# ml-jku/LRAM

Measured on AMD Instinct MI355X. Metric: env-steps/sec (action-inference), higher is better.
Workload: dtype f32

## Files before the change

lram_amd/csrc/engine.h:

```cpp
#pragma once
#include <algorithm>
#include <array>
#include <cstdlib>
#include <cstring>
#include <map>
#include <memory>
#include <string>
#include <vector>

#include "../../include/lram_hip.h"
#include "common.h"

namespace lram::host {

struct DevBuf {
  float* p = nullptr;
  size_t n = 0;
  void alloc(size_t numel) {
    release();
    if (numel == 0) return;
    LRAM_HIP_CHECK(hipMalloc(reinterpret_cast<void**>(&p), numel * sizeof(float)));
    n = numel;
  }
  void zero(hipStream_t s = nullptr) {
    if (p) LRAM_HIP_CHECK(hipMemsetAsync(p, 0, n * sizeof(float), s));
  }
  void release() {
    if (p) (void)hipFree(p);
    p = nullptr;
    n = 0;
  }
};

struct BlockWeights {
  const float *norm_g = nullptr, *norm_b = nullptr;
  const float *proj_up = nullptr, *conv_w = nullptr, *conv_b = nullptr, *wq = nullptr, *wk = nullptr, *wv = nullptr,
              *wi = nullptr, *bi = nullptr, *wf = nullptr, *bf = nullptr, *on_g = nullptr, *on_b = nullptr,
              *skip = nullptr, *proj_down = nullptr;
  const float *gate_w[4] = {nullptr, nullptr, nullptr, nullptr};
  const float *rt = nullptr, *rbias = nullptr, *gn_g = nullptr, *gn_b = nullptr, *ffn_norm_g = nullptr,
              *ffn_norm_b = nullptr, *ffn_up = nullptr, *ffn_down = nullptr;
  const float *in_proj = nullptr, *in_proj_b = nullptr, *x_proj = nullptr, *dt_proj = nullptr, *dt_bias = nullptr,
              *A_log = nullptr, *Dp = nullptr, *out_proj = nullptr, *out_proj_b = nullptr;
};

struct BlockState {
  DevBuf s0;
  DevBuf n;
  DevBuf m;
  DevBuf conv;
  DevBuf wk, wv;
  DevBuf coef;
  DevBuf gsc;
  DevBuf pw;
};

struct GraphKey {
  const void *obs, *rtg, *rew, *mask, *act, *tok;
  int emb, discrete, B;
  hipStream_t stream;
  bool operator==(const GraphKey& o) const {
    return obs == o.obs && rtg == o.rtg && rew == o.rew && mask == o.mask && act == o.act && tok == o.tok &&
           emb == o.emb && discrete == o.discrete && B == o.B && stream == o.stream;
  }
};

}

using namespace lram;
using namespace lram::host;

constexpr int kTokenTapMaxBatch = 1024;

struct lram_engine {
  lram_config cfg{};
  int device = 0;
  std::map<std::string, DevBuf> weights;
  bool finalized = false;
  std::vector<BlockWeights> bw;
  struct Split {
    uint16_t* p;
    size_t n;
  };
  std::map<const float*, Split> split;
  bool use_bf16x3 = true;
  bool use_f16x2 = true;
  int f16x2_min_rows = 256;
  struct Split16 {
    uint16_t* planes;
    float* inv;
    size_t rows, k;
  };
  std::map<const float*, Split16> split16;
  bool gemm_presplit = true;
  int64_t slstm_counts[3] = {0, 0, 0};
  double gemm_counts[8] = {0, 0, 0, 0, 0, 0, 0, 0};
  std::vector<DevBuf> slstm_rt2;
  std::vector<DevBuf> slstm_rinv;
  int lazy_cap2_envs = 896;
  std::map<const float*, DevBuf> narrow;
  bool gemm_narrow_on = true;
  int gemm_narrow_min_rows = 256;
  bool upz_beside = true;
  bool slstm_gates_one = true;
  bool gemm_narrow_f16 = true;
  bool gn_amax_handover = true;
  bool gn_planes = true;
  bool slstm_seq_f32 = false;
  bool slstm_seq = true;
  std::vector<DevBuf> gate_coef;
  bool front_multi = true;
  int front_min_envs = 256;
  std::vector<DevBuf> dt_wt;
  DevBuf ASCALE;
  size_t ascale_rows = 0;
  DevBuf AMX_XN, AMX_XA, AMX_H;
  const float *w_state = nullptr, *b_state = nullptr, *w_rtg = nullptr, *b_rtg = nullptr, *w_rew = nullptr,
              *b_rew = nullptr, *eln_g = nullptr, *eln_b = nullptr, *w_head = nullptr, *b_head = nullptr,
              *post_g = nullptr, *post_b = nullptr;
  struct ImgConv {
    const float *w = nullptr, *b = nullptr;
    int cin = 0, cout = 0;
  };
  ImgConv img_conv[3][5];
  const float *img_lin_w = nullptr, *img_lin_b = nullptr;
  int img_channels = 0, img_flat = 0;
  DevBuf IMG_P, IMG_X0, IMG_X1, IMG_T;
  DevBuf IMG_EMB;
  DevBuf IMG_FLAT, IMG_ROWS, IMG_LIST;
  int img_tile = 2048;
  int64_t img_counts[3] = {0, 0, 0};
  static constexpr int fold_bubbles_images = 8;
  bool slot_table = false;
  std::vector<uint8_t> slot_flags, slot_act;
  std::vector<int32_t> slot_img_prefix;
  uint8_t* slot_dev = nullptr;
  int32_t* slot_img_list = nullptr;
  int slot_n_image = 0;
  bool slot_has_discrete = false;
  int mask_words = 0;
  std::vector<uint32_t> mask_bits;
  uint32_t* mask_dev = nullptr;
  int mask_no_discrete_at = -1;
  static int mask_count_below(const uint32_t* bits, int words, int b, int n) {
    int cnt = 0;
    for (int k = 0; k < words && k * 32 < n; ++k) {
      const int left = n - k * 32;
      cnt += __builtin_popcount(bits[(size_t)b * words + k] & (left >= 32 ? 0xffffffffu : (1u << left) - 1u));
    }
    return cnt;
  }
  int mask_first_empty(const uint32_t* bits, int words, const uint8_t* flags) const {
    for (int b = 0; b < B; ++b) {
      const int n = (flags != nullptr && (flags[b] & 1)) ? cfg.n_discrete : cfg.n_vocab;
      if (mask_count_below(bits, words, b, n) == 0) return b;
    }
    return -1;
  }
  void drop_action_mask() {
    if (mask_dev) (void)hipFree(mask_dev);
    mask_dev = nullptr, mask_words = 0, mask_no_discrete_at = -1;
    mask_bits.clear();
  }
  int lazy_mode = 2;
  bool lazy = false;
  bool lazy_ready = false;
  int lazy_period = 13;
  int gn_fuse = 2;
  bool mamba_dt_fuse = true;
  int slstm_fused_rows = 512;
  int gemm_skinny_rows = 384;
  static constexpr int slstm_gates_rows = 768;
  int gemm_skinny_min = 5;
  static constexpr int gemm_skinny_k = 1024;
  static constexpr int fold_bubbles = 2;
  bool fold_tail = true;
  static constexpr int fold_tail_blocks = 2;
  struct Prefold {
    bool pending = false;
    int blocks = 0;
    int64_t step = 0;
    int period = 0, B = 0;
  } prefold;
  int64_t lazy_step = 0;
  std::vector<int> lazy_bound;
  bool lazy_dirty = false;
  DevBuf LZ_COUNT;
  std::vector<SlotSeg> slot_segs;
  SlotSeg* slot_segs_dev = nullptr;
  SlotChunk* slot_chunks_dev = nullptr;
  int slot_n_chunks = 0, slot_n_rec_chunks = 0;
  int32_t* slot_idx_dev = nullptr;
  std::vector<int64_t> slot_c_off;
  bool slot_y_checked = false;
  void drop_slot_segments() {
    if (slot_segs_dev) (void)hipFree(slot_segs_dev);
    if (slot_chunks_dev) (void)hipFree(slot_chunks_dev);
    if (slot_idx_dev) (void)hipFree(slot_idx_dev);
    slot_segs_dev = nullptr, slot_chunks_dev = nullptr, slot_idx_dev = nullptr;
    slot_segs.clear(), slot_c_off.clear();
    slot_n_chunks = slot_n_rec_chunks = 0;
  }
  int B = 0;
  int n_live = 0;
  int ctx_rows = 0;
  int context_rows() const { return ctx_rows == 0 ? B : n_live; }
  int64_t ctx_counts[4] = {0, 0, 0, 0};
  int64_t parked_dirty_step = 0;
  bool parked_windows_empty(int64_t step) const { return step - parked_dirty_step >= (int64_t)lazy_period; }
  std::vector<BlockState> st;
  DevBuf X, XN, TOK, HID, U, Q, K, V, XA, H, G, SCAL, RY, LOGITS, RES, DTP;
  DevBuf XN2;
  DevBuf GATES, AMAT, VEC;
  DevBuf SEQ_EMB;
  DevBuf CTX, KEEP;
  DevBuf SCORE_LG;
  int score_rows = 4096;
  static constexpr int kScoreMinRows = 16;
  int last_head = -1;
  int tok_cap = 0;
  bool chunk_prefill = true;
  bool chunk_exact_fp32 = false;
  bool chunk_lanes = true;
  static constexpr int kMaxLanes = 3;
  static constexpr int n_lanes = 3;
  DevBuf twin[kMaxLanes - 1][21];
  std::vector<hipEvent_t> lane_ev[kMaxLanes];
  DevBuf SK;
  static constexpr size_t kSplitKSlotElems = 6u << 20;
  static constexpr int kSplitKSlots = 9;
  size_t ucols = 0, icols = 0;
  bool graph_mode = false;
  bool graph_valid = false;
  GraphKey graph_key{};
  hipGraph_t graph = nullptr;
  hipGraphExec_t graph_exec = nullptr;
  hipStream_t capture_stream = nullptr;
  int n_micro = 0;
  int compat_repeat = 1;
  DevBuf X0, U0;
  bool compat_share = true;
  bool compat_stale = false;
  bool sampling = false;
  SampleArgs sample;
  uint64_t* sample_draw = nullptr;
  std::vector<SampleSlot> sample_slots;
  SampleSlot* sample_slots_dev = nullptr;
  int sslot_k_max = 0, sslot_k_at = -1, sslot_kd_max = 0, sslot_kd_at = -1;
  void sample_slot_maxima() {
    sslot_k_max = sslot_kd_max = 0, sslot_k_at = sslot_kd_at = -1;
    for (size_t b = 0; b < sample_slots.size(); ++b) {
      const SampleSlot& t = sample_slots[b];
      if (t.mode == 0) continue;
      if (t.top_k > sslot_k_max) sslot_k_max = t.top_k, sslot_k_at = (int)b;
      if (slot_table && b < slot_flags.size() && (slot_flags[b] & 1) && t.top_k > sslot_kd_max)
        sslot_kd_max = t.top_k, sslot_kd_at = (int)b;
    }
  }
  void drop_sample_slots() {
    if (sample_slots_dev) (void)hipFree(sample_slots_dev);
    sample_slots_dev = nullptr;
    sample_slots.clear();
    sample_slot_maxima();
  }
  static constexpr int cell_unroll = 16;
// ... 207 lines not shown
```

lram_amd/csrc/engine.hip:

```cpp
#include "engine.h"

namespace {

const float* need(lram_engine* e, const std::string& name, size_t numel) {
  auto it = e->weights.find(name);
  if (it == e->weights.end()) throw Error("lram: missing weight '" + name + "'");
  if (it->second.n != numel)
    throw Error("lram: weight '" + name + "' has " + std::to_string(it->second.n) + " elements, expected " +
                std::to_string(numel));
  return it->second.p;
}
const float* optional(lram_engine* e, const std::string& name, size_t numel) {
  auto it = e->weights.find(name);
  if (it == e->weights.end()) return nullptr;
  if (it->second.n != numel)
    throw Error("lram: weight '" + name + "' has " + std::to_string(it->second.n) + " elements, expected " +
                std::to_string(numel));
  return it->second.p;
}

void validate_config(const lram_config& c) {
  LRAM_REQUIRE(c.abi_version == LRAM_ABI_VERSION, "config.abi_version does not match the library");
  LRAM_REQUIRE(c.backbone == LRAM_BACKBONE_XLSTM || c.backbone == LRAM_BACKBONE_MAMBA, "unknown backbone");
  LRAM_REQUIRE(c.d_model > 0 && c.d_model % 4 == 0 && c.d_model <= 2048, "d_model must be a multiple of 4, <= 2048");
// ... 326 lines not shown
                        (size_t)e->B * c.n_heads * (kChunkMaxTokens + 3) * kChunkMaxTokens * 4;
    if (want > have + free_b - std::min<size_t>(free_b, (size_t)2 << 30)) return seq;
    alloc_workspace(e, kChunkMaxTokens);
    LRAM_HIP_CHECK(hipDeviceSynchronize());
  }
  return steps;
}

}

namespace {

bool lazy_geometry_ok(const lram_engine* e) {
  return has_mlstm_block(e) && mlstm_lazy_supported(e->cfg.inner / e->cfg.n_heads, e->cfg.tokens_per_step);
}

void slot_segments_build(lram_engine* e) {
  e->drop_slot_segments();
  if (e->B <= 0) return;
  const lram_config& c = e->cfg;
  const int64_t B = e->B;
  std::vector<SlotSeg>& segs = e->slot_segs;
  int64_t rec = 0;
  const int64_t rec_numel = lram_state_bytes_per_env(e) / 4;
  auto add = [&](float* base, int64_t stride, int64_t numel, int kind, int parity, bool in_record) {
    if (base == nullptr || numel <= 0) return;
    SlotSeg sg{};
    sg.base = base, sg.stride = stride, sg.numel = (int32_t)numel, sg.kind = kind, sg.parity = parity;
    sg.rec_off = in_record ? rec : -1;
    const bool slot_ok = numel % 4 == 0 && stride % 4 == 0 && (reinterpret_cast<uintptr_t>(base) & 15) == 0;
    const bool rec_ok = in_record && rec % 4 == 0 && rec_numel % 4 == 0;
    sg.vec = (slot_ok ? 1 : 0) | (slot_ok && rec_ok ? 2 : 0);
    if (in_record) rec += numel;
    segs.push_back(sg);
  };
  e->slot_c_off.assign(c.n_blocks, -1);
  e->slot_y_checked = false;
  for (int i = 0; i < c.n_blocks; ++i) {
    BlockState& s = e->st[i];
    if (c.backbone == LRAM_BACKBONE_MAMBA) {
      add(s.s0.p, (int64_t)c.d_inner * c.d_state, (int64_t)c.d_inner * c.d_state, kSlotSegState, -1, true);
      add(s.conv.p, (int64_t)c.d_inner * c.d_conv, (int64_t)c.d_inner * c.d_conv, kSlotSegState, -1, true);
    } else if (c.block_is_slstm[i]) {
      const int64_t D = c.d_model;
      const bool checked = e->slstm_rinv.size() > (size_t)i && e->slstm_rinv[i].p != nullptr;
      e->slot_y_checked = e->slot_y_checked || checked;
      for (int p = 0; p < 4; ++p)
        add(s.s0.p + p * B * D, D, D, p == 0 && checked ? kSlotSegSlstmY : kSlotSegState, -1, true);
      add(s.conv.p, (int64_t)c.conv_k * D, (int64_t)c.conv_k * D, kSlotSegState, -1, true);
    } else {
      const int64_t NH = c.n_heads, DH = e->dh();
      e->slot_c_off[i] = rec;
      add(s.s0.p, NH * DH * DH, NH * DH * DH, kSlotSegC, -1, true);
      add(s.n.p, c.inner, c.inner, kSlotSegState, -1, true);
      add(s.m.p, NH, NH, kSlotSegState, -1, true);
      add(s.conv.p, (int64_t)c.conv_k * c.inner, (int64_t)c.conv_k * c.inner, kSlotSegState, -1, true);
    }
  }
  LRAM_REQUIRE(rec == rec_numel, "slot state: the segment table does not add up to the record size");
  const size_t n_rec_segs = segs.size();
  if (e->lazy_ready) {
    const int64_t NH = c.n_heads, DH = e->dh(), W = kLazyWindow;
    for (int i = 0; i < c.n_blocks; ++i) {
      if (c.block_is_slstm[i]) continue;
      BlockState& s = e->st[i];
      add(s.wk.p, NH * W * DH, NH * W * DH, kSlotSegWindow, -1, false);
      add(s.wv.p, NH * W * DH, NH * W * DH, kSlotSegWindow, -1, false);
      for (int p = 0; p < 2; ++p) {
        add(s.coef.p + p * B * NH * W, NH * W, NH * W, kSlotSegCoef, p, false);
        add(s.gsc.p + p * B * NH, NH, NH, kSlotSegG, p, false);
      }
    }
    for (int p = 0; p < 2; ++p) add(e->LZ_COUNT.p + p * B, 1, 1, kSlotSegCount, p, false);
  }
  std::vector<SlotChunk> chunks;
  for (size_t k = 0; k < segs.size(); ++k) {
    if (k == n_rec_segs) e->slot_n_rec_chunks = (int)chunks.size();
    for (int32_t off = 0; off < segs[k].numel; off += kSlotChunk) chunks.push_back(SlotChunk{(int32_t)k, off});
  }
  if (segs.size() == n_rec_segs) e->slot_n_rec_chunks = (int)chunks.size();
  e->slot_n_chunks = (int)chunks.size();
  LRAM_HIP_CHECK(hipMalloc(reinterpret_cast<void**>(&e->slot_segs_dev), segs.size() * sizeof(SlotSeg)));
  LRAM_HIP_CHECK(hipMalloc(reinterpret_cast<void**>(&e->slot_chunks_dev), chunks.size() * sizeof(SlotChunk)));
  LRAM_HIP_CHECK(hipMalloc(reinterpret_cast<void**>(&e->slot_idx_dev), 2 * (size_t)B * sizeof(int32_t)));
  LRAM_HIP_CHECK(hipMemcpy(e->slot_segs_dev, segs.data(), segs.size() * sizeof(SlotSeg), hipMemcpyHostToDevice));
  LRAM_HIP_CHECK(hipMemcpy(e->slot_chunks_dev, chunks.data(), chunks.size() * sizeof(SlotChunk), hipMemcpyHostToDevice));
}

void lazy_alloc(lram_engine* e) {
  if (e->lazy_ready || e->B <= 0 || !lazy_geometry_ok(e)) return;
  const lram_config& c = e->cfg;
  const size_t B = e->B, NH = c.n_heads, DH = e->dh();
  for (int i = 0; i < c.n_blocks; ++i) {
    if (c.block_is_slstm[i]) continue;
    BlockState& s = e->st[i];
    s.wk.alloc(B * NH * kLazyWindow * DH);
    s.wv.alloc(B * NH * kLazyWindow * DH);
    s.coef.alloc(2 * B * NH * kLazyWindow);
    s.gsc.alloc(2 * B * NH);
    if (!mlstm_lazy_fused_scores((int)DH)) {
      s.pw.alloc(B * NH * 4 * kLazyWT);
      s.pw.zero();
    }
    s.coef.zero();
  }
  e->LZ_COUNT.alloc(2 * B);
  e->LZ_COUNT.zero();
  for (int i = 0; i < c.n_blocks; ++i) {
    if (c.block_is_slstm[i]) continue;
    BlockState& s = e->st[i];
    for (int p = 0; p < 2; ++p)
      launch_mlstm_lazy_clear(reinterpret_cast<int32_t*>(e->LZ_COUNT.p) + p * B, s.gsc.p + p * B * NH, nullptr, (int)B,
                              (int)NH, nullptr);
  }
  LRAM_HIP_CHECK(hipDeviceSynchronize());
  e->lazy_step = 0;
  e->parked_dirty_step = 0;
  e->prefold = lram_engine::Prefold{};
  e->lazy_ready = true;
  slot_segments_build(e);
}

bool lazy_choice(const lram_engine* e) {
  if (e->lazy_mode == 0 || !lazy_geometry_ok(e)) return false;
  if (e->lazy_mode == 1) return true;
  return mlstm_block_bytes(e) >= 128.0 * 1024 * 1024;
}

struct Knob {
  const char* name;
  void (*set)(lram_engine& e, const char* v);
};
const Knob kKnobs[] = {
    {"LRAM_STATE", [](lram_engine& e, const char* v) {
       const std::string m(v);
       e.lazy_mode = m == "lazy" ? 1 : (m == "eager" || m == "materialised" || m == "materialized") ? 0 : 2;
     }},
    {"LRAM_LAZY_PERIOD", [](lram_engine& e, const char* v) { e.lazy_period = std::max(1, std::min(14, std::atoi(v))); }},
    {"LRAM_LAZY_CAP2_ENVS", [](lram_engine& e, const char* v) { e.lazy_cap2_envs = std::max(0, std::atoi(v)); }},
    {"LRAM_FOLD_TAIL", [](lram_engine& e, const char* v) { e.fold_tail = std::atoi(v) != 0; }},
    {"LRAM_GN_FUSE", [](lram_engine& e, const char* v) { e.gn_fuse = std::max(0, std::min(2, std::atoi(v))); }},
    {"LRAM_F16_MIN_ROWS", [](lram_engine& e, const char* v) { e.f16x2_min_rows = std::max(9, std::atoi(v)); }},
    {"LRAM_GEMM_PRESPLIT", [](lram_engine& e, const char* v) { e.gemm_presplit = std::atoi(v) != 0; }},
    {"LRAM_GEMM_NARROW", [](lram_engine& e, const char* v) { e.gemm_narrow_on = std::atoi(v) != 0, e.gemm_narrow_f16 = std::atoi(v) != 2; }},
    {"LRAM_UPZ_8P", [](lram_engine& e, const char* v) { e.upz_beside = std::atoi(v) != 0; }},
    {"LRAM_SLSTM_GATES_ONE", [](lram_engine& e, const char* v) { e.slstm_gates_one = std::atoi(v) != 0; }},
    {"LRAM_GN_AMAX", [](lram_engine& e, const char* v) { e.gn_amax_handover = std::atoi(v) != 0, e.gn_planes = std::atoi(v) >= 2; }},
    {"LRAM_GEMM_SKINNY_ROWS", [](lram_engine& e, const char* v) { e.gemm_skinny_rows = std::max(0, std::atoi(v)); }},
    {"LRAM_GEMM_SKINNY_MIN", [](lram_engine& e, const char* v) { e.gemm_skinny_min = std::max(1, std::atoi(v)); }},
    {"LRAM_SLSTM_FUSED_ROWS", [](lram_engine& e, const char* v) { e.slstm_fused_rows = std::max(0, std::atoi(v)); }},
    {"LRAM_SLSTM_SEQ", [](lram_engine& e, const char* v) { e.slstm_seq = std::atoi(v) != 0, e.slstm_seq_f32 = std::atoi(v) == 2; }},
    {"LRAM_FRONT_MULTI", [](lram_engine& e, const char* v) { e.front_multi = std::atoi(v) != 0; }},
    {"LRAM_FRONT_MIN_ENVS", [](lram_engine& e, const char* v) { e.front_min_envs = std::max(1, std::atoi(v)); }},
    {"LRAM_MAMBA_DT_FUSE", [](lram_engine& e, const char* v) { e.mamba_dt_fuse = std::atoi(v) != 0; }},
    {"LRAM_COMPAT_SHARE", [](lram_engine& e, const char* v) { e.compat_share = std::atoi(v) != 0; }},
    {"LRAM_PREFILL_CHUNK", [](lram_engine& e, const char* v) {
       e.chunk_prefill = std::atoi(v) != 0, e.chunk_exact_fp32 = std::atoi(v) == 2, e.chunk_lanes = std::atoi(v) != 3;
     }},
    {"LRAM_SCORE_ROWS", [](lram_engine& e, const char* v) { e.score_rows = std::max(lram_engine::kScoreMinRows, std::atoi(v)); }},
    {"LRAM_IMG_TILE", [](lram_engine& e, const char* v) { e.img_tile = std::max(1, std::min(kConvMaxFrames, std::atoi(v))); }},
    {"LRAM_EVENT_SCOPE", [](lram_engine& e, const char* v) { e.event_device_scope = std::string(v) != "system"; }},
};

void state_alloc(lram_engine* e, int B) {
  LRAM_REQUIRE(e->finalized, "lram_finalize must be called before lram_state_alloc");
  LRAM_REQUIRE(B > 0 && B <= 65535, "batch must be in 1..65535");
  LRAM_HIP_CHECK(hipSetDevice(e->device));
  e->drop_graph();
  e->release_state();
  e->drop_slot_table();
  e->drop_sample_slots();
  e->drop_action_mask();
  const lram_config& c = e->cfg;
  const size_t D = c.d_model;
  e->st.resize(c.n_blocks);
  for (int i = 0; i < c.n_blocks; ++i) {
    BlockState& s = e->st[i];
    if (c.backbone == LRAM_BACKBONE_MAMBA) {
      s.s0.alloc((size_t)B * c.d_inner * c.d_state);
      s.conv.alloc((size_t)B * c.d_inner * c.d_conv);
    } else if (c.block_is_slstm[i]) {
      s.s0.alloc(4 * (size_t)B * D);
      s.conv.alloc((size_t)B * c.conv_k * D);
    } else {
      const size_t DH = e->dh();
      s.s0.alloc((size_t)B * c.n_heads * DH * DH);
      s.n.alloc((size_t)B * c.inner);
      s.m.alloc((size_t)B * c.n_heads);
      s.conv.alloc((size_t)B * c.conv_k * c.inner);
    }
    s.s0.zero();
    s.n.zero();
    s.m.zero();
    s.conv.zero();
  }
  e->B = B;
  e->n_live = B;
  e->ctx_rows = LRAM_CONTEXT_ROWS_ALL;
  alloc_workspace(e, kMaxTokens);
  e->lazy = lazy_choice(e);
  if (e->lazy) lazy_alloc(e);
  if (e->slot_segs_dev == nullptr) slot_segments_build(e);
  LRAM_HIP_CHECK(hipDeviceSynchronize());
}

}

extern "C" {

const char* lram_last_error(void) { return g_last_error.c_str(); }

int32_t lram_abi_version(void) { return LRAM_ABI_VERSION; }

int32_t lram_create(const lram_config* cfg, int32_t device, lram_engine** out) {
  return guarded([&] {
    LRAM_REQUIRE(cfg != nullptr && out != nullptr, "lram_create: null argument");
    validate_config(*cfg);
    int ndev = 0;
    LRAM_HIP_CHECK(hipGetDeviceCount(&ndev));
    LRAM_REQUIRE(device >= 0 && device < ndev, "lram_create: no such HIP device");
    LRAM_HIP_CHECK(hipSetDevice(device));
    auto e = std::make_unique<lram_engine>();
    e->cfg = *cfg;
    e->device = device;
    gemm_knobs_reload();
    for (const Knob& k : kKnobs)
      if (const char* v = std::getenv(k.name)) k.set(*e, v);
    *out = e.release();
  });
}

int32_t lram_destroy(lram_engine* e) {
  return guarded([&] {
    if (e) {
      (void)hipSetDevice(e->device);
      delete e;
    }
  });
}

int32_t lram_set_weight(lram_engine* e, const char* name, const float* host_data, size_t numel) {
  return guarded([&] {
    LRAM_REQUIRE(e && name && host_data && numel > 0, "lram_set_weight: bad argument");
    LRAM_HIP_CHECK(hipSetDevice(e->device));
    DevBuf& b = e->weights[name];
    b.alloc(numel);
    LRAM_HIP_CHECK(hipMemcpy(b.p, host_data, numel * sizeof(float), hipMemcpyHostToDevice));
    e->finalized = false;
    e->drop_graph();
  });
}

int32_t lram_finalize(lram_engine* e) {
  return guarded([&] {
    LRAM_REQUIRE(e != nullptr, "lram_finalize: null engine");
    finalize(e);
  });
}

int32_t lram_state_alloc(lram_engine* e, int32_t batch) {
  return guarded([&] {
    LRAM_REQUIRE(e != nullptr, "lram_state_alloc: null engine");
    state_alloc(e, batch);
  });
}

int64_t lram_state_bytes_per_env(const lram_engine* e) {
  if (!e) return 0;
  const lram_config& c = e->cfg;
  int64_t elems = 0;
  for (int i = 0; i < c.n_blocks; ++i) {
    if (c.backbone == LRAM_BACKBONE_MAMBA) {
      elems += (int64_t)c.d_inner * (c.d_state + c.d_conv);
    } else if (c.block_is_slstm[i]) {
      elems += (int64_t)c.d_model * (4 + c.conv_k);
    } else {
      const int64_t DH = c.inner / c.n_heads;
      elems += (int64_t)c.n_heads * DH * DH + c.inner + c.n_heads + (int64_t)c.conv_k * c.inner;
    }
  }
  return elems * 4;
}

int32_t lram_set_graph_mode(lram_engine* e, int32_t enable) {
  return guarded([&] {
    LRAM_REQUIRE(e != nullptr, "lram_set_graph_mode: null engine");
    if (e->prefold.pending || (enable != 0 && e->lazy_ready)) {
      LRAM_HIP_CHECK(hipSetDevice(e->device));
      LRAM_HIP_CHECK(hipDeviceSynchronize());
      if (enable != 0)
        lazy_materialize(e, nullptr);
      else
        lazy_finish_prefold(e, nullptr);
      LRAM_HIP_CHECK(hipDeviceSynchronize());
    }
    e->graph_mode = enable != 0;
    if (!e->graph_mode) e->drop_graph();
  });
}

int32_t lram_set_state_mode(lram_engine* e, int32_t mode, int32_t fold_period) {
  return guarded([&] {
    LRAM_REQUIRE(e != nullptr, "lram_set_state_mode: null engine");
    LRAM_REQUIRE(mode >= 0 && mode <= 2, "lram_set_state_mode: mode must be 0 (materialised), 1 (lazy) or 2 (auto)");
    LRAM_REQUIRE(fold_period == 0 || (fold_period >= 1 && fold_period * e->cfg.tokens_per_step + 4 <= kLazyWindow),
                 "lram_set_state_mode: fold_period out of range (the window holds 48 tokens)");
// ... 158 lines not shown
```

lram_amd/csrc/engine_xlstm.hip:

```cpp
#include "engine.h"

namespace {

MlstmLazyArgs lazy_args(lram_engine* e, int i, int T, const uint8_t* reset, int b0, int nb, int step_off = 0) {
  const lram_config& c = e->cfg;
  const size_t NH = c.n_heads, DH = e->dh(), B = e->B;
  const int64_t step = e->lazy_step + step_off;
  const int in = (int)(step & 1), out = 1 - in;
  BlockState& st = e->st[i];
  MlstmLazyArgs a{};
  a.C = st.s0.p + (size_t)b0 * NH * DH * DH;
  a.wk = st.wk.p + (size_t)b0 * NH * kLazyWindow * DH;
  a.wv = st.wv.p + (size_t)b0 * NH * kLazyWindow * DH;
  a.coef_in = st.coef.p + (in * B + b0) * NH * kLazyWindow;
  a.coef_out = st.coef.p + (out * B + b0) * NH * kLazyWindow;
  a.g_in = st.gsc.p + (in * B + b0) * NH;
  a.g_out = st.gsc.p + (out * B + b0) * NH;
  a.count_in = reinterpret_cast<const int32_t*>(e->LZ_COUNT.p) + in * B + b0;
  a.count_out = reinterpret_cast<int32_t*>(e->LZ_COUNT.p) + out * B + b0;
  a.pw = st.pw.p ? st.pw.p + (size_t)b0 * NH * T * kLazyWT : nullptr;
  a.reset = reset ? reset + b0 : nullptr;
  a.B = nb, a.T = T, a.NH = (int)NH, a.DH = (int)DH;
  a.phase = (int)((step + b0) % e->lazy_period), a.period = e->lazy_period, a.force = 0;
  return a;
}

bool lazy_bound_compact(const lram_engine* e, int64_t step, int T) {
  const int P = e->lazy_period;
  if ((int)e->lazy_bound.size() != P) return false;
  const int c_due = lazy_due_class(step, P);
  for (int cls = 0; cls < P; ++cls)
    if (cls != c_due && e->lazy_bound[cls] + T > kLazyWindow) return false;
  return true;
}

void fold_block(lram_engine* e, int i, int T, const uint8_t* reset, bool compact, int step_off, hipStream_t s) {
  MlstmLazyArgs la = lazy_args(e, i, T, reset, 0, e->n_live, step_off);
  la.compact = compact ? 1 : 0;
  prof_record(e, s, true, true);
  launch_mlstm_lazy_fold(la, s);
  if (e->n_live < e->B && !e->parked_windows_empty(e->lazy_step + step_off)) {
    MlstmLazyArgs lp = lazy_args(e, i, T, nullptr, e->n_live, e->B - e->n_live, step_off);
    lp.compact = compact ? 2 : 0;
    launch_mlstm_lazy_fold(lp, s);
  }
  prof_record(e, s, false, true);
}

}

namespace lram::host {

void lazy_materialize(lram_engine* e, hipStream_t s) {
  lazy_finish_prefold(e, s);
  if (!e->lazy_ready || !e->lazy_dirty) return;
  const lram_config& c = e->cfg;
  const size_t B = e->B, NH = c.n_heads;
  for (int i = 0; i < c.n_blocks; ++i) {
    if (c.block_is_slstm[i]) continue;
    MlstmLazyArgs a = lazy_args(e, i, 1, nullptr, 0, e->B);
    a.force = 1;
    launch_mlstm_lazy_fold(a, s);
  }
  for (int i = 0; i < c.n_blocks; ++i) {
    if (c.block_is_slstm[i]) continue;
    for (int p = 0; p < 2; ++p)
      launch_mlstm_lazy_clear(reinterpret_cast<int32_t*>(e->LZ_COUNT.p) + p * B, e->st[i].gsc.p + p * B * NH, nullptr,
                              (int)B, (int)NH, s);
  }
  e->lazy_bound.assign(e->lazy_period, 0);
  e->lazy_dirty = false;
}

void lazy_finish_prefold(lram_engine* e, hipStream_t s) {
  if (!e->prefold.pending) return;
  const lram_engine::Prefold pf = e->prefold;
  e->prefold = lram_engine::Prefold{};
  LRAM_REQUIRE(e->lazy_ready && pf.B == e->B && pf.period == e->lazy_period && pf.step == e->lazy_step,
               "lazy mLSTM: a tail fold is pending for another state than the engine holds");
  const lram_config& c = e->cfg;
  const int B = e->B, NH = c.n_heads, P = e->lazy_period;
  const int side = (int)(e->lazy_step & 1);
  const int first = lazy_due_class(e->lazy_step, P);
  int k = 0;
  for (int i = 0; i < c.n_blocks; ++i) {
    if (c.block_is_slstm[i] || k++ < pf.blocks) continue;
    MlstmLazyArgs a = lazy_args(e, i, 1, nullptr, 0, B);
    a.compact = 1;
    launch_mlstm_lazy_fold(a, s);
  }
  int32_t* count = reinterpret_cast<int32_t*>(e->LZ_COUNT.p) + (size_t)side * B;
  for (int i = 0; i < c.n_blocks; ++i)
    if (!c.block_is_slstm[i]) launch_mlstm_lazy_folded(count, e->st[i].gsc.p + (size_t)side * B * NH, B, NH, first, P, s);
  launch_mlstm_lazy_folded(count, nullptr, B, NH, first, P, s);
  if ((int)e->lazy_bound.size() == P) e->lazy_bound[first] = 0;
}

}

namespace {

bool lean_front(const lram_engine* e, int T) {
  return lazy_active(e, T) && mlstm_lazy_fused_scores(e->cfg.inner / e->cfg.n_heads);
}

bool split_up_now(const lram_engine* e) { return e->n_live >= 2048 && !e->graph_mode; }

bool gn_fused(const lram_engine* e, int T) {
  const int dh = e->cfg.inner / e->cfg.n_heads;
  return (e->gn_fuse == 1 || (e->gn_fuse == 2 && e->n_live >= 2048)) && lean_front(e, T) && e->use_bf16x3 && (dh == 256 || dh == 128) && T <= 4 &&
         e->cfg.inner % 8 == 0 && e->cfg.d_model % 8 == 0 && e->n_live >= 64;
}

void mlstm_front(lram_engine* e, const Pass& pass, int i, int T, const uint8_t* reset, const Slice& sl) {
  const lram_config& c = e->cfg;
  const int D = c.d_model, inner = c.inner, NH = c.n_heads, rows = sl.nb * T;
  const size_t r0 = (size_t)sl.b0 * T, b0 = sl.b0;
  const BlockWeights& w = e->bw[i];
  BlockState& st = e->st[i];
  float* amx = e->use_f16x2 ? e->AMX_XN.p + r0 : nullptr;
  GemmArgs up;
  up.a = e->XN.p + r0 * D, up.lda = D, up.w = w.proj_up, up.ldw = D, up.c = e->U.p + r0 * e->ucols, up.ldc = 2 * inner;
  up.m = rows, up.n = split_up_now(e) ? inner : 2 * inner, up.k = D;
  if (gn_fused(e, T) && !split_up_now(e)) up.act_silu_from = inner;
  if (!split_up_now(e) && takes_skinny_with_norm(e, up)) {
    up.a = e->X.p + r0 * D, up.norm_g = w.norm_g, up.norm_b = w.norm_b, up.norm_eps = c.ln_eps, up.norm_rms = c.norm_is_rms;
    launch_gemm_skinny(up, sl.s);
    count_gemm(e, 3, up);
  } else {
    const bool ps = presplit_for(e, w.proj_up, rows, inner, D);
    uint16_t* xn2 = reinterpret_cast<uint16_t*>(e->XN2.p) + r0 * 32;
    const int64_t xn2_kt = ps ? (int64_t)(e->XN2.n / D) * 32 : 0;
    launch_row_norm(e->X.p + r0 * D, D, ps ? nullptr : e->XN.p + r0 * D, D, w.norm_g, w.norm_b, rows, D, c.ln_eps,
                    c.norm_is_rms, sl.s, nullptr, ps ? nullptr : amx, nullptr, ps ? xn2 : nullptr, (int64_t)e->XN2.n,
                    ps ? amx : nullptr, xn2_kt);
    up.a_amax = amx;
    if (ps) up.a = nullptr, up.a_amax = nullptr, up.a2 = xn2, up.a2_plane = (int64_t)e->XN2.n, up.a2_kt = xn2_kt, up.a2_inv = amx;
    if (pass.lane_rec != nullptr) up.beside_memory_bound = 2;
    gemm(e, up, sl.s);
  }
  if (e->front_multi && lean_front(e, T) && sl.nb >= e->front_min_envs && e->gate_coef[i].p != nullptr &&
      mlstm_front_supported(inner, NH, c.conv_k, T)) {
    MlstmFrontArgs fa;
    fa.u = e->U.p + r0 * e->ucols, fa.ldu = 2 * inner, fa.conv_state = st.conv.p + b0 * c.conv_k * inner;
    fa.n_state = st.n.p + b0 * inner, fa.m_state = st.m.p + b0 * NH;
    fa.conv_w = w.conv_w, fa.conv_b = w.conv_b, fa.wq = w.wq, fa.wk = w.wk, fa.gc = e->gate_coef[i].p, fa.bi = w.bi, fa.bf = w.bf;
    fa.xa = e->XA.p + r0 * e->icols, fa.scal = e->SCAL.p + r0 * NH * 4, fa.reset = reset ? reset + b0 : nullptr;
    fa.B = sl.nb, fa.T = T, fa.inner = inner, fa.NH = NH, fa.K = c.conv_k;
    LRAM_REQUIRE(pass.hold == nullptr, "mLSTM front end: the multi-env kernel has no hold rule (stored contexts run materialised)");
    launch_mlstm_front(fa, sl.s);
    return;
  }
  MlstmPreArgs pa;
  pa.u = e->U.p + r0 * e->ucols, pa.conv_state = st.conv.p + b0 * c.conv_k * inner, pa.n_state = st.n.p + b0 * inner;
  pa.m_state = st.m.p + b0 * NH;
  pa.conv_w = w.conv_w, pa.conv_b = w.conv_b, pa.wq = w.wq, pa.wk = w.wk, pa.wv = w.wv;
  pa.wi = w.wi, pa.bi = w.bi, pa.wf = w.wf, pa.bf = w.bf;
  pa.q = e->Q.p + r0 * e->icols, pa.k = e->K.p + r0 * e->icols, pa.v = e->V.p + r0 * e->icols;
  pa.xa = e->XA.p + r0 * e->icols;
  pa.scal = e->SCAL.p + r0 * NH * 4, pa.reset = reset ? reset + b0 : nullptr;
  pa.hold = pass.hold ? pass.hold + b0 : nullptr;
  pa.B = sl.nb, pa.T = T, pa.inner = inner, pa.NH = NH, pa.K = c.conv_k;
  pa.lean = lean_front(e, T) ? 1 : 0;
  if (T > kMaxTokens) {
    LRAM_REQUIRE(T <= e->tok_cap && e->AMAT.p != nullptr, "chunkwise prefill workspace not allocated");
    pa.gates = e->GATES.p + r0 * NH * 2;
    pa.amat = e->AMAT.p + b0 * NH * kChunkMaxTokens * kChunkMaxTokens;
    pa.vec = e->VEC.p + b0 * NH * 3 * kChunkMaxTokens;
  }
  launch_mlstm_pre(pa, sl.s);
}

void mlstm_up_z(lram_engine* e, int i, int T, const Slice& sl) {
  if (!split_up_now(e)) return;
  const lram_config& c = e->cfg;
  const int D = c.d_model, inner = c.inner, rows = sl.nb * T;
  const size_t r0 = (size_t)sl.b0 * T;
  GemmArgs up;
  up.a = e->XN.p + r0 * D, up.lda = D, up.w = e->bw[i].proj_up + (size_t)inner * D, up.ldw = D;
  up.c = e->U.p + r0 * e->ucols + inner, up.ldc = 2 * inner, up.m = rows, up.n = inner, up.k = D;
  if (e->use_f16x2) up.a_amax = e->AMX_XN.p + r0;
  if (presplit_for(e, e->bw[i].proj_up, rows, inner, D)) {
    up.a = nullptr, up.a_amax = nullptr;
    up.a2 = reinterpret_cast<uint16_t*>(e->XN2.p) + r0 * 32, up.a2_plane = (int64_t)e->XN2.n, up.a2_kt = (int64_t)(e->XN2.n / D) * 32;
    up.a2_inv = e->AMX_XN.p + r0;
  }
  if (gn_fused(e, T)) up.act_silu_from = 0;
  up.beside_memory_bound = e->upz_beside ? 1 : 0;
  gemm(e, up, sl.s);
}

void mlstm_cell(lram_engine* e, const Pass& pass, int i, int T, const uint8_t* reset, const Slice& sl, hipStream_t s) {
  const lram_config& c = e->cfg;
  const int inner = c.inner, NH = c.n_heads, DH = e->dh();
  const size_t r0 = (size_t)sl.b0 * T, b0 = sl.b0;
  MlstmCellArgs ca;
  ca.C = e->st[i].s0.p + b0 * NH * DH * DH, ca.q = e->Q.p + r0 * e->icols, ca.k = e->K.p + r0 * e->icols;
  ca.v = e->V.p + r0 * e->icols, ca.scal = e->SCAL.p + r0 * NH * 4, ca.h = e->H.p + r0 * e->icols;
  ca.reset = reset ? reset + b0 : nullptr, ca.B = sl.nb, ca.T = T, ca.NH = NH, ca.DH = DH;
  ca.hold = pass.hold ? pass.hold + b0 : nullptr;
  const long wgs = (long)sl.nb * NH * ((DH % 256 == 0) ? DH / 256 : (DH % 128 == 0) ? DH / 128 : DH / 64);
  ca.min_lds_bytes = wgs >= 1024 ? 84 * 1024 : 0;
  ca.unroll = e->cell_unroll;
  if (T > kMaxTokens) {
    ca.amat = e->AMAT.p + b0 * NH * kChunkMaxTokens * kChunkMaxTokens;
    ca.vec = e->VEC.p + b0 * NH * 3 * kChunkMaxTokens;
    ca.chunk_exact_fp32 = e->chunk_exact_fp32 ? 1 : 0;
  }
  prof_record(e, s, true);
  launch_mlstm_cell(ca, s);
  prof_record(e, s, false);
}

void mlstm_back(lram_engine* e, const Pass& pass, int i, int T, const Slice& sl) {
  const lram_config& c = e->cfg;
  const int D = c.d_model, inner = c.inner, NH = c.n_heads, DH = e->dh(), rows = sl.nb * T;
  const size_t r0 = (size_t)sl.b0 * T;
  const BlockWeights& w = e->bw[i];
  float* X = e->X.p + r0 * D;
  if (gn_fused(e, T)) {
    GemmArgs dn;
    dn.a = e->H.p + r0 * e->icols, dn.lda = inner, dn.w = w.proj_down, dn.ldw = inner, dn.c = X, dn.ldc = D, dn.residual = X;
    dn.m = rows, dn.n = D, dn.k = inner;
    dn.gate = e->U.p + r0 * e->ucols + inner, dn.ldg = 2 * inner;
    gemm(e, dn, sl.s);
    return;
  }
  GroupNormArgs ga;
  ga.h = e->H.p + r0 * e->icols, ga.gamma = w.on_g, ga.beta = w.on_b, ga.skip = w.skip, ga.xa = e->XA.p + r0 * e->icols;
  ga.u = e->U.p + r0 * e->ucols, ga.out = e->G.p + r0 * e->icols, ga.rows = rows, ga.NH = NH, ga.DH = DH, ga.mode = 0;
  ga.eps = c.ln_eps;
  const bool hand_over = e->gn_amax_handover && e->AMX_H.p != nullptr && f16x2_rows(e, rows, D, inner);
  GemmArgs dn;
  dn.a = e->G.p + r0 * e->icols, dn.lda = inner, dn.w = w.proj_down, dn.ldw = inner, dn.c = X, dn.ldc = D, dn.residual = X;
  dn.m = rows, dn.n = D, dn.k = inner;
  const int64_t bt = (int64_t)(e->G.n / e->icols);
  GemmArgs probe;
  const bool planes = hand_over && e->gn_planes && pass.n_slices == 1 && e->gemm_presplit && NH <= 8 && (inner & 31) == 0 && bt * inner * 4 < (1ll << 31) &&
                      f16x2_weight(e, w.proj_down, inner, &probe) && 4 * probe.w2_plane < (1ll << 31);
  if (planes) {
    ga.out = nullptr;
    ga.h2 = reinterpret_cast<uint16_t*>(e->G.p) + r0 * 32, ga.h2_plane = bt * inner, ga.h2_kt = bt * 32, ga.h2_inv = e->AMX_H.p + r0;
    dn.a = nullptr, dn.a2 = ga.h2, dn.a2_plane = ga.h2_plane, dn.a2_kt = ga.h2_kt, dn.a2_inv = ga.h2_inv;
  } else {
    ga.amax = hand_over ? e->AMX_H.p + r0 * NH : nullptr;
    if (hand_over) dn.a_amax = ga.amax, dn.amax_parts = NH;
  }
  launch_group_norm(ga, sl.s);
  gemm(e, dn, sl.s);
}

bool slstm_gates_one_bf16x3(const lram_engine* e, GemmArgs& g4, const BlockWeights& w, const float* XC, const float* XN, float* gates,
                            int Hs) {
  if (!e->use_bf16x3 || !e->slstm_gates_one) return false;
  int64_t plane = -1;
  for (int g = 0; g < 4; ++g) {
    auto it = e->split.find(w.gate_w[g]);
    if (it == e->split.end() || (plane >= 0 && (int64_t)it->second.n != plane)) return false;
    plane = (int64_t)it->second.n;
    g4.a_tab[g] = (g < 2) ? XC : XN, g4.w_tab[g] = w.gate_w[g], g4.c_tab[g] = gates + (int64_t)g * Hs;
    g4.w3_tab[g] = it->second.p;
  }
  g4.w3 = g4.w3_tab[0], g4.w3_plane = plane;
  return gemm_bf16x3_supported(g4) && !gemm_small_m(g4);
}

void slstm_block(lram_engine* e, const Pass& pass, int i, int T, const uint8_t* reset, const Slice& sl) {
  const lram_config& c = e->cfg;
  const int D = c.d_model, NH = c.n_heads, SDH = e->sdh(), F = c.ffn_dim, Hs = D, rows = sl.nb * T;
  const size_t r0 = (size_t)sl.b0 * T, b0 = sl.b0;
  const BlockWeights& w = e->bw[i];
  BlockState& st = e->st[i];
  hipStream_t s = sl.s;
  float* X = e->X.p + r0 * D;
  float* XN = e->XN.p + r0 * D;
  float* XC = e->Q.p + r0 * e->icols;
  float* gates = e->U.p + r0 * e->ucols;
  float* RY = e->RY.p + b0 * 4 * Hs;
  float* Y = e->H.p + r0 * e->icols;
  float* Ubuf = e->U.p + r0 * e->ucols;
  float* Gbuf = e->G.p + r0 * e->icols;
  float* state = st.s0.p + b0 * Hs;
  const uint8_t* hold = pass.hold ? pass.hold + b0 : nullptr;
  launch_row_norm(X, D, XN, D, w.norm_g, w.norm_b, rows, D, c.ln_eps, c.norm_is_rms, s);
  SlstmConvArgs sa;
  sa.xn = XN, sa.conv_state = st.conv.p + b0 * c.conv_k * D, sa.slstm_state = state, sa.conv_w = w.conv_w;
  sa.conv_b = w.conv_b, sa.xc = XC, sa.reset = reset ? reset + b0 : nullptr, sa.B = sl.nb, sa.T = T, sa.D = D;
  sa.K = c.conv_k, sa.state_B = e->B, sa.hold = hold;
  launch_slstm_conv(sa, s);
  GemmArgs g4;
  g4.a = XC, g4.lda = D, g4.sA1 = SDH, g4.w = w.gate_w[0], g4.ldw = SDH, g4.sW1 = (int64_t)SDH * SDH;
  g4.c = gates, g4.ldc = 4 * Hs, g4.sC1 = SDH, g4.m = rows, g4.n = SDH, g4.k = SDH, g4.nb1 = NH, g4.nb2 = 4;
  const bool gates_big = rows <= e->slstm_gates_rows && gemm_skinny_supported(g4) && g4.k <= 128;
  bool tab_aligned = true;
  for (int g = 0; g < 4; ++g)
    tab_aligned = tab_aligned && ((reinterpret_cast<uintptr_t>((g < 2) ? XC : XN) | reinterpret_cast<uintptr_t>(w.gate_w[g])) & 15) == 0;
  if (tab_aligned && (takes_skinny(e, g4) || gates_big)) {
    for (int g = 0; g < 4; ++g)
      g4.a_tab[g] = (g < 2) ? XC : XN, g4.w_tab[g] = w.gate_w[g], g4.c_tab[g] = gates + (int64_t)g * Hs;
    launch_gemm_skinny(g4, s);
    count_gemm(e, 3, g4);
// ... 225 lines not shown
```

lram_amd/csrc/mlstm_front.hip:

```cpp
#include <algorithm>
#include <cstdlib>

#include "common.h"
#include "device_math.h"
#include "xlstm_rules.h"

namespace lram {

namespace {

__global__ __launch_bounds__(256) void gate_coef_kernel(const float* wq, const float* wk, const float* wv, const float* wi,
                                                        const float* wf, int inner, int NH, float* gc) {
  const int gid = blockIdx.x * blockDim.x + threadIdx.x;
  const int ngroups = inner >> 2;
  if (gid >= ngroups * 2 * NH * 4) return;
  const int c = gid & 3, j = (gid >> 2) % (2 * NH), cg = gid / (8 * NH);
  const float* wg = (j < NH ? wi + (int64_t)j * 3 * inner : wf + (int64_t)(j - NH) * 3 * inner) + 4 * cg;
  double a = 0.0, b = 0.0;
  for (int o = 0; o < 4; ++o) {
    a += (double)wg[o] * (double)wq[(int64_t)cg * 16 + o * 4 + c] + (double)wg[inner + o] * (double)wk[(int64_t)cg * 16 + o * 4 + c];
    b += (double)wg[2 * inner + o] * (double)wv[(int64_t)cg * 16 + o * 4 + c];
  }
  gc[((int64_t)cg * 4 * NH + j) * 4 + c] = (float)a;
  gc[((int64_t)cg * 4 * NH + 2 * NH + j) * 4 + c] = (float)b;
}

template <int N, int M>
__device__ __forceinline__ void halve(const float* v, float* r, int lane) {
  const bool up = (lane & M) != 0;
#pragma unroll
  for (int i = 0; i < N; ++i) {
    const float send = up ? v[i] : v[i + N];
    const float keep = up ? v[i + N] : v[i];
    r[i] = keep + __shfl_xor(send, M, 64);
  }
}

constexpr int kNH = 4;
constexpr int kNG = 2 * kNH;

template <int T>
__global__ __launch_bounds__(256) void mlstm_front_kernel(MlstmFrontArgs a) {
  static_assert(T == 3, "the reduction tree below is laid out for 3 tokens x 8 gates");
  __shared__ float red[2][4][T * kNG];
  const int tid = threadIdx.x, lane = tid & 63, wave = tid >> 6;
  const int inner = 4 * 256, c0 = tid << 2, h = wave;
  const int e_begin = blockIdx.x * a.epw, e_end = min(a.B, e_begin + a.epw);
  if (e_begin >= e_end) return;

  float4 cw[4], wq[4], wk[4], gc[2 * kNG];
#pragma unroll
  for (int c = 0; c < 4; ++c) cw[c] = *reinterpret_cast<const float4*>(a.conv_w + (int64_t)(c0 + c) * 4);
  const float4 cb = *reinterpret_cast<const float4*>(a.conv_b + c0);
#pragma unroll
  for (int o = 0; o < 4; ++o) {
    wq[o] = *reinterpret_cast<const float4*>(a.wq + (int64_t)tid * 16 + o * 4);
    wk[o] = *reinterpret_cast<const float4*>(a.wk + (int64_t)tid * 16 + o * 4);
  }
#pragma unroll
  for (int j = 0; j < 2 * kNG; ++j) gc[j] = *reinterpret_cast<const float4*>(a.gc + ((int64_t)tid * 2 * kNG + j) * 4);
  const float bias_i = a.bi[h], bias_f = a.bf[h];
  const float sqrt_dh = 16.f;

  float4 win[4], nst, xm[T];
  float m_in;
  unsigned rsb;
  const uint8_t* rbase = a.reset != nullptr ? a.reset : reinterpret_cast<const uint8_t*>(a.conv_w);
  auto request = [&](int b) {
#pragma unroll
    for (int k = 0; k < 4; ++k) win[k] = *reinterpret_cast<const float4*>(a.conv_state + ((int64_t)b * 4 + k) * inner + c0);
    nst = *reinterpret_cast<const float4*>(a.n_state + (int64_t)b * inner + c0);
#pragma unroll
    for (int t = 0; t < T; ++t) xm[t] = *reinterpret_cast<const float4*>(a.u + ((int64_t)b * T + t) * a.ldu + c0);
    m_in = a.m_state[(int64_t)b * kNH + h];
    rsb = rbase[a.reset != nullptr ? b : 0];
  };
  request(e_begin);

  for (int b = e_begin; b < e_end; ++b) {
    const int buf = (b - e_begin) & 1;
    const unsigned keep = (a.reset != nullptr && rsb != 0) ? 0u : 0xFFFFFFFFu;
    float4 w0 = masked4(win[0], keep), w1 = masked4(win[1], keep), w2 = masked4(win[2], keep), w3 = masked4(win[3], keep);
    float4 n = masked4(nst, keep);
    float m = masked(m_in, keep);
    const float4 x0 = xm[0], x1 = xm[1], x2 = xm[2];

    float4 q[T], k[T];
    float pg[T * kNG];
    auto token = [&](int t, const float4& p0, const float4& p1, const float4& p2, const float4& p3) {
      const float4 xa = conv4_silu(p0, p1, p2, p3, cw, cb);
      *reinterpret_cast<float4*>(a.xa + ((int64_t)b * T + t) * inner + c0) = xa;
      q[t] = block4x4(wq, xa);
      k[t] = block4x4(wk, xa);
#pragma unroll
      for (int j = 0; j < kNG; ++j) pg[t * kNG + j] = dot4(gc[j], xa) + dot4(gc[kNG + j], p3);
    };
    token(0, w1, w2, w3, x0);
    token(1, w2, w3, x0, x1);
    token(2, w3, x0, x1, x2);
    *reinterpret_cast<float4*>(a.conv_state + ((int64_t)b * 4 + 0) * inner + c0) = w3;
    *reinterpret_cast<float4*>(a.conv_state + ((int64_t)b * 4 + 1) * inner + c0) = x0;
    *reinterpret_cast<float4*>(a.conv_state + ((int64_t)b * 4 + 2) * inner + c0) = x1;
    *reinterpret_cast<float4*>(a.conv_state + ((int64_t)b * 4 + 3) * inner + c0) = x2;

    request(min(b + 1, e_end - 1));

    float r12[12], r6[6], r3[3];
    halve<12, 32>(pg, r12, lane);
    halve<6, 16>(r12, r6, lane);
    halve<3, 8>(r6, r3, lane);
#pragma unroll
    for (int i = 0; i < 3; ++i) {
      r3[i] += __shfl_xor(r3[i], 4, 64);
      r3[i] += __shfl_xor(r3[i], 2, 64);
      r3[i] += __shfl_xor(r3[i], 1, 64);
    }
    if ((lane & 7) == 0) {
      const int idx = ((lane & 32) ? 12 : 0) + ((lane & 16) ? 6 : 0) + ((lane & 8) ? 3 : 0);
#pragma unroll
      for (int i = 0; i < 3; ++i) red[buf][wave][idx + i] = r3[i];
    }
    __syncthreads();

    float f[T], ig[T], mt[T];
#pragma unroll
    for (int t = 0; t < T; ++t) {
      const float gi = red[buf][0][t * kNG + h] + red[buf][1][t * kNG + h] + red[buf][2][t * kNG + h] + red[buf][3][t * kNG + h] + bias_i;
      const float gf = red[buf][0][t * kNG + kNH + h] + red[buf][1][t * kNG + kNH + h] + red[buf][2][t * kNG + kNH + h] +
                       red[buf][3][t * kNG + kNH + h] + bias_f;
      const MlstmGate g = mlstm_gate_step(gi, gf, m);
      f[t] = g.f;
      ig[t] = g.i;
      mt[t] = m = g.m;
    }
    float d[T];
#pragma unroll
    for (int t = 0; t < T; ++t) {
      n = mlstm_n_step(n, f[t], ig[t], k[t], sqrt_dh);
      d[t] = wave_sum(dot4(q[t], n));
    }
    *reinterpret_cast<float4*>(a.n_state + (int64_t)b * inner + c0) = n;
    if (lane == 0) {
      a.m_state[(int64_t)b * kNH + h] = m;
#pragma unroll
      for (int t = 0; t < T; ++t) {
        *reinterpret_cast<float4*>(a.scal + (((int64_t)b * T + t) * kNH + h) * 4) =
            make_float4(f[t], ig[t], mlstm_denominator(d[t], mt[t]), mt[t]);
      }
    }
  }
}

}

bool mlstm_front_supported(int inner, int NH, int K, int T) { return inner == 1024 && NH == kNH && K == 4 && T == 3; }

void launch_gate_coef(const float* wq, const float* wk, const float* wv, const float* wi, const float* wf, int inner, int NH,
                      float* gc, hipStream_t stream) {
  const int n = (inner >> 2) * 2 * NH * 4;
  hipLaunchKernelGGL(gate_coef_kernel, dim3((unsigned)((n + 255) / 256)), dim3(256), 0, stream, wq, wk, wv, wi, wf, inner, NH, gc);
  LRAM_HIP_CHECK(hipGetLastError());
}

void launch_mlstm_front(const MlstmFrontArgs& a_in, hipStream_t stream) {
  MlstmFrontArgs a = a_in;
  LRAM_REQUIRE(mlstm_front_supported(a.inner, a.NH, a.K, a.T), "mLSTM multi-env front end: unsupported geometry");
  LRAM_REQUIRE(a.gc != nullptr && (a.ldu & 3) == 0, "mLSTM multi-env front end: missing gate coefficients / misaligned u");
  static const int epw_env = [] {
    const char* v = std::getenv("LRAM_FRONT_EPW");
    return v ? std::atoi(v) : 0;
  }();
  a.epw = epw_env > 0 ? epw_env : (a.epw > 0 ? a.epw : std::max(1, std::min(8, a.B / 256)));
  const int nwg = (a.B + a.epw - 1) / a.epw;
  hipLaunchKernelGGL(mlstm_front_kernel<3>, dim3((unsigned)nwg), dim3(256), 0, stream, a);
  LRAM_HIP_CHECK(hipGetLastError());
}

}
```

Measured before the change: 464,700.

## Cut mLSTM front-end register pressure via shared gate coefs and wave-uniform addressing

Restructures the multi-env mLSTM front kernel to hold fewer values in registers. Half of the gate coefficients now live in shared memory. The q/k weights and the other half of the gate coefficients are reloaded for each env instead of being kept resident. Row pointers and gate scalars are made wave-uniform with readfirstlane so the compiler can use scalar address registers. The epw override moves from a static getenv to an engine setting. The aim is higher occupancy, paid for with extra per-env reloads, which should mostly hit cache.

Measured after the change: 463,100. No clear change (-0.3%).

```diff
diff --git a/lram_amd/csrc/engine.h b/lram_amd/csrc/engine.h
--- a/lram_amd/csrc/engine.h
+++ b/lram_amd/csrc/engine.h
@@ -111,6 +111,7 @@
   std::vector<DevBuf> gate_coef;
   bool front_multi = true;
   int front_min_envs = 256;
+  int front_epw = 0;
   std::vector<DevBuf> dt_wt;
   DevBuf ASCALE;
   size_t ascale_rows = 0;
diff --git a/lram_amd/csrc/engine.hip b/lram_amd/csrc/engine.hip
--- a/lram_amd/csrc/engine.hip
+++ b/lram_amd/csrc/engine.hip
@@ -502,6 +502,7 @@
     {"LRAM_SLSTM_SEQ", [](lram_engine& e, const char* v) { e.slstm_seq = std::atoi(v) != 0, e.slstm_seq_f32 = std::atoi(v) == 2; }},
     {"LRAM_FRONT_MULTI", [](lram_engine& e, const char* v) { e.front_multi = std::atoi(v) != 0; }},
     {"LRAM_FRONT_MIN_ENVS", [](lram_engine& e, const char* v) { e.front_min_envs = std::max(1, std::atoi(v)); }},
+    {"LRAM_FRONT_EPW", [](lram_engine& e, const char* v) { e.front_epw = std::max(0, std::atoi(v)); }},
     {"LRAM_MAMBA_DT_FUSE", [](lram_engine& e, const char* v) { e.mamba_dt_fuse = std::atoi(v) != 0; }},
     {"LRAM_COMPAT_SHARE", [](lram_engine& e, const char* v) { e.compat_share = std::atoi(v) != 0; }},
     {"LRAM_PREFILL_CHUNK", [](lram_engine& e, const char* v) {
diff --git a/lram_amd/csrc/engine_xlstm.hip b/lram_amd/csrc/engine_xlstm.hip
--- a/lram_amd/csrc/engine_xlstm.hip
+++ b/lram_amd/csrc/engine_xlstm.hip
@@ -146,7 +146,7 @@
     fa.n_state = st.n.p + b0 * inner, fa.m_state = st.m.p + b0 * NH;
     fa.conv_w = w.conv_w, fa.conv_b = w.conv_b, fa.wq = w.wq, fa.wk = w.wk, fa.gc = e->gate_coef[i].p, fa.bi = w.bi, fa.bf = w.bf;
     fa.xa = e->XA.p + r0 * e->icols, fa.scal = e->SCAL.p + r0 * NH * 4, fa.reset = reset ? reset + b0 : nullptr;
-    fa.B = sl.nb, fa.T = T, fa.inner = inner, fa.NH = NH, fa.K = c.conv_k;
+    fa.B = sl.nb, fa.T = T, fa.inner = inner, fa.NH = NH, fa.K = c.conv_k, fa.epw = e->front_epw;
     LRAM_REQUIRE(pass.hold == nullptr, "mLSTM front end: the multi-env kernel has no hold rule (stored contexts run materialised)");
     launch_mlstm_front(fa, sl.s);
     return;
diff --git a/lram_amd/csrc/mlstm_front.hip b/lram_amd/csrc/mlstm_front.hip
--- a/lram_amd/csrc/mlstm_front.hip
+++ b/lram_amd/csrc/mlstm_front.hip
@@ -1,5 +1,4 @@
 #include <algorithm>
-#include <cstdlib>
 
 #include "common.h"
 #include "device_math.h"
@@ -39,40 +38,59 @@
 constexpr int kNH = 4;
 constexpr int kNG = 2 * kNH;
 
+constexpr int kFrontThreads = 256;
+
+template <class E>
+__device__ __forceinline__ __attribute__((address_space(1))) E* uniform_row(const E* row) {
+  const uint64_t v = reinterpret_cast<uint64_t>(row);
+  const uint32_t lo = __builtin_amdgcn_readfirstlane((uint32_t)v), hi = __builtin_amdgcn_readfirstlane((uint32_t)(v >> 32));
+  return reinterpret_cast<__attribute__((address_space(1))) E*>(((uint64_t)hi << 32) | lo);
+}
+__device__ __forceinline__ float wave_uniform(float v) { return __uint_as_float(__builtin_amdgcn_readfirstlane(__float_as_uint(v))); }
+__device__ __forceinline__ float4 row_ld4(const float* row, unsigned c) {
+  const v4f v = uniform_row(reinterpret_cast<const v4f*>(row))[c >> 2];
+  return make_float4(v.x, v.y, v.z, v.w);
+}
+__device__ __forceinline__ void row_st4(float* row, unsigned c, const float4& v) {
+  uniform_row(reinterpret_cast<const v4f*>(row))[c >> 2] = v4f{v.x, v.y, v.z, v.w};
+}
+
 template <int T>
-__global__ __launch_bounds__(256) void mlstm_front_kernel(MlstmFrontArgs a) {
+__global__ __launch_bounds__(kFrontThreads) void mlstm_front_kernel(MlstmFrontArgs a) {
   static_assert(T == 3, "the reduction tree below is laid out for 3 tokens x 8 gates");
   __shared__ float red[2][4][T * kNG];
+  __shared__ float4 gcx[kNG][kFrontThreads];
   const int tid = threadIdx.x, lane = tid & 63, wave = tid >> 6;
-  const int inner = 4 * 256, c0 = tid << 2, h = wave;
+  const int inner = 4 * 256, h = wave;
+  const unsigned c0 = tid << 2;
   const int e_begin = blockIdx.x * a.epw, e_end = min(a.B, e_begin + a.epw);
   if (e_begin >= e_end) return;
 
-  float4 cw[4], wq[4], wk[4], gc[2 * kNG];
+  float4 cw[4], gc[kNG];
 #pragma unroll
   for (int c = 0; c < 4; ++c) cw[c] = *reinterpret_cast<const float4*>(a.conv_w + (int64_t)(c0 + c) * 4);
   const float4 cb = *reinterpret_cast<const float4*>(a.conv_b + c0);
 #pragma unroll
-  for (int o = 0; o < 4; ++o) {
-    wq[o] = *reinterpret_cast<const float4*>(a.wq + (int64_t)tid * 16 + o * 4);
-    wk[o] = *reinterpret_cast<const float4*>(a.wk + (int64_t)tid * 16 + o * 4);
-  }
-#pragma unroll
-  for (int j = 0; j < 2 * kNG; ++j) gc[j] = *reinterpret_cast<const float4*>(a.gc + ((int64_t)tid * 2 * kNG + j) * 4);
-  const float bias_i = a.bi[h], bias_f = a.bf[h];
+  for (int j = 0; j < kNG; ++j) gcx[j][tid] = *reinterpret_cast<const float4*>(a.gc + ((int64_t)tid * 2 * kNG + kNG + j) * 4);
+  auto request_gc = [&]() {
+#pragma unroll
+    for (int j = 0; j < kNG; ++j) gc[j] = row_ld4(a.gc + j * 4, c0 << 4);
+  };
+  request_gc();
+  const float bias_i = wave_uniform(a.bi[h]), bias_f = wave_uniform(a.bf[h]);
   const float sqrt_dh = 16.f;
-
-  float4 win[4], nst, xm[T];
+  __syncthreads();
+
+  float4 win[3], xm[T];
   float m_in;
   unsigned rsb;
   const uint8_t* rbase = a.reset != nullptr ? a.reset : reinterpret_cast<const uint8_t*>(a.conv_w);
   auto request = [&](int b) {
 #pragma unroll
-    for (int k = 0; k < 4; ++k) win[k] = *reinterpret_cast<const float4*>(a.conv_state + ((int64_t)b * 4 + k) * inner + c0);
-    nst = *reinterpret_cast<const float4*>(a.n_state + (int64_t)b * inner + c0);
-#pragma unroll
-    for (int t = 0; t < T; ++t) xm[t] = *reinterpret_cast<const float4*>(a.u + ((int64_t)b * T + t) * a.ldu + c0);
-    m_in = a.m_state[(int64_t)b * kNH + h];
+    for (int k = 0; k < 3; ++k) win[k] = row_ld4(a.conv_state + ((int64_t)b * 4 + k + 1) * inner, c0);
+#pragma unroll
+    for (int t = 0; t < T; ++t) xm[t] = row_ld4(a.u + ((int64_t)b * T + t) * a.ldu, c0);
+    m_in = *uniform_row(a.m_state + (int64_t)b * kNH + h);
     rsb = rbase[a.reset != nullptr ? b : 0];
   };
   request(e_begin);
@@ -80,28 +98,30 @@
   for (int b = e_begin; b < e_end; ++b) {
     const int buf = (b - e_begin) & 1;
     const unsigned keep = (a.reset != nullptr && rsb != 0) ? 0u : 0xFFFFFFFFu;
-    float4 w0 = masked4(win[0], keep), w1 = masked4(win[1], keep), w2 = masked4(win[2], keep), w3 = masked4(win[3], keep);
-    float4 n = masked4(nst, keep);
+    float4 w1 = masked4(win[0], keep), w2 = masked4(win[1], keep), w3 = masked4(win[2], keep);
     float m = masked(m_in, keep);
     const float4 x0 = xm[0], x1 = xm[1], x2 = xm[2];
 
-    float4 q[T], k[T];
+    float4 xa[T];
     float pg[T * kNG];
     auto token = [&](int t, const float4& p0, const float4& p1, const float4& p2, const float4& p3) {
-      const float4 xa = conv4_silu(p0, p1, p2, p3, cw, cb);
-      *reinterpret_cast<float4*>(a.xa + ((int64_t)b * T + t) * inner + c0) = xa;
-      q[t] = block4x4(wq, xa);
-      k[t] = block4x4(wk, xa);
-#pragma unroll
-      for (int j = 0; j < kNG; ++j) pg[t * kNG + j] = dot4(gc[j], xa) + dot4(gc[kNG + j], p3);
+      xa[t] = conv4_silu(p0, p1, p2, p3, cw, cb);
+      row_st4(a.xa + ((int64_t)b * T + t) * inner, c0, xa[t]);
     };
     token(0, w1, w2, w3, x0);
     token(1, w2, w3, x0, x1);
     token(2, w3, x0, x1, x2);
-    *reinterpret_cast<float4*>(a.conv_state + ((int64_t)b * 4 + 0) * inner + c0) = w3;
-    *reinterpret_cast<float4*>(a.conv_state + ((int64_t)b * 4 + 1) * inner + c0) = x0;
-    *reinterpret_cast<float4*>(a.conv_state + ((int64_t)b * 4 + 2) * inner + c0) = x1;
-    *reinterpret_cast<float4*>(a.conv_state + ((int64_t)b * 4 + 3) * inner + c0) = x2;
+#pragma unroll
+    for (int j = 0; j < kNG; ++j) {
+      const float4 gx = gcx[j][tid];
+      pg[0 * kNG + j] = dot4(gc[j], xa[0]) + dot4(gx, x0);
+      pg[1 * kNG + j] = dot4(gc[j], xa[1]) + dot4(gx, x1);
+      pg[2 * kNG + j] = dot4(gc[j], xa[2]) + dot4(gx, x2);
+    }
+    row_st4(a.conv_state + ((int64_t)b * 4 + 0) * inner, c0, w3);
+    row_st4(a.conv_state + ((int64_t)b * 4 + 1) * inner, c0, x0);
+    row_st4(a.conv_state + ((int64_t)b * 4 + 2) * inner, c0, x1);
+    row_st4(a.conv_state + ((int64_t)b * 4 + 3) * inner, c0, x2);
 
     request(min(b + 1, e_end - 1));
 
@@ -119,6 +139,13 @@
       const int idx = ((lane & 32) ? 12 : 0) + ((lane & 16) ? 6 : 0) + ((lane & 8) ? 3 : 0);
 #pragma unroll
       for (int i = 0; i < 3; ++i) red[buf][wave][idx + i] = r3[i];
+    }
+    float4 wq[4], wk[4];
+    float4 n = masked4(row_ld4(a.n_state + (int64_t)b * inner, c0), keep);
+#pragma unroll
+    for (int o = 0; o < 4; ++o) {
+      wq[o] = row_ld4(a.wq + o * 4, c0 << 2);
+      wk[o] = row_ld4(a.wk + o * 4, c0 << 2);
     }
     __syncthreads();
 
@@ -129,23 +156,26 @@
       const float gf = red[buf][0][t * kNG + kNH + h] + red[buf][1][t * kNG + kNH + h] + red[buf][2][t * kNG + kNH + h] +
                        red[buf][3][t * kNG + kNH + h] + bias_f;
       const MlstmGate g = mlstm_gate_step(gi, gf, m);
-      f[t] = g.f;
-      ig[t] = g.i;
-      mt[t] = m = g.m;
-    }
+      f[t] = wave_uniform(g.f);
+      ig[t] = wave_uniform(g.i);
+      mt[t] = m = wave_uniform(g.m);
+    }
+    float4 q[T], k[T];
+#pragma unroll
+    for (int t = 0; t < T; ++t) q[t] = block4x4(wq, xa[t]), k[t] = block4x4(wk, xa[t]);
+    request_gc();
     float d[T];
 #pragma unroll
     for (int t = 0; t < T; ++t) {
       n = mlstm_n_step(n, f[t], ig[t], k[t], sqrt_dh);
       d[t] = wave_sum(dot4(q[t], n));
     }
-    *reinterpret_cast<float4*>(a.n_state + (int64_t)b * inner + c0) = n;
+    row_st4(a.n_state + (int64_t)b * inner, c0, n);
     if (lane == 0) {
-      a.m_state[(int64_t)b * kNH + h] = m;
+      *uniform_row(a.m_state + (int64_t)b * kNH + h) = m;
 #pragma unroll
       for (int t = 0; t < T; ++t) {
-        *reinterpret_cast<float4*>(a.scal + (((int64_t)b * T + t) * kNH + h) * 4) =
-            make_float4(f[t], ig[t], mlstm_denominator(d[t], mt[t]), mt[t]);
+        row_st4(a.scal + (((int64_t)b * T + t) * kNH + h) * 4, 0, make_float4(f[t], ig[t], mlstm_denominator(d[t], mt[t]), mt[t]));
       }
     }
   }
@@ -166,11 +196,7 @@
   MlstmFrontArgs a = a_in;
   LRAM_REQUIRE(mlstm_front_supported(a.inner, a.NH, a.K, a.T), "mLSTM multi-env front end: unsupported geometry");
   LRAM_REQUIRE(a.gc != nullptr && (a.ldu & 3) == 0, "mLSTM multi-env front end: missing gate coefficients / misaligned u");
-  static const int epw_env = [] {
-    const char* v = std::getenv("LRAM_FRONT_EPW");
-    return v ? std::atoi(v) : 0;
-  }();
-  a.epw = epw_env > 0 ? epw_env : (a.epw > 0 ? a.epw : std::max(1, std::min(8, a.B / 256)));
+  a.epw = a.epw > 0 ? a.epw : std::max(1, std::min(8, a.B / 256));
   const int nwg = (a.B + a.epw - 1) / a.epw;
   hipLaunchKernelGGL(mlstm_front_kernel<3>, dim3((unsigned)nwg), dim3(256), 0, stream, a);
   LRAM_HIP_CHECK(hipGetLastError());
```
